# pr0g/ToyMeshPathTracer

Measured on AMD Instinct MI355X. Metric: MRays/s on sponza.obj 1920x1080 64spp at 1/2/4/8 GPUs; %HBM roofline, higher is better.
Workload: dtype f32

## Files before the change

toymeshpathtracer_amd/csrc/tmpt_aov.hip:

```cpp
#include <hip/hip_runtime.h>

#include <algorithm>
#include <string>

#include "tmpt_render.h"

namespace tmpt {

static_assert(sizeof(tmpt_aov_pixel) == 32, "AOV record: two 16-byte stores");

constexpr int kAovTicket = 8;

struct AovSample {
    f3 n;
    float t, lc;
    uint32_t flags;
    int32_t tri;
};

template <int BLOCK, int SL>
__device__ __forceinline__ AovSample aov_sample(const SceneView& sv, const RenderArgs& a, uint32_t x, uint32_t y,
                                                uint32_t smp, uint32_t& rays, uint32_t& srays,
                                                TravStack<BLOCK, SL>& st, TravCount& cnt)
{
// ... 107 lines not shown
{
    auto fn = k_aov<G, kBlk, kSL>;
    const int resident = occupancy_grid((const void*)fn, kBlk, 0, s.device);
    int grid = (int)std::max<int64_t>(1, std::min<int64_t>(resident, (a.slots * G + kBlk - 1) / kBlk));
    const size_t ovf_bytes = (size_t)grid * kBlk * (kStackTotal - kSL) * sizeof(uint32_t);
    if (ensure_ws(s, ovf_bytes)) return -1;
    fn<<<grid, kBlk, 0, s.stream>>>(view(s), a, reinterpret_cast<float4*>(d_out), (uint32_t*)s.ws, s.counters);
    TMPT_HIP(hipGetLastError());
    return 0;
}

int render_aov(Scene& s, const tmpt_camera* cam, const tmpt_render_desc* d, tmpt_aov_pixel* d_out,
               uint64_t* ray_count)
{
    RenderArgs a = make_args(cam, d);
    s.row_render = false;
    if (int rc = ensure_sample_tables(s, a.spp, "tmpt_render_aov")) return rc;
    a.jt = s.jt;
    if (int rc = wait_caller_stream(s, d, "tmpt_render_aov")) return rc;
    if (ensure_counters(s)) return -1;
    a.root_check = camera_root_check(s, a.cam);
    TMPT_HIP(hipMemsetAsync(s.counters, 0, kRenderCounters * sizeof(unsigned long long), s.stream));
    hipEvent_t e0 = s.render_ev[0], e1 = s.render_ev[1];
    TMPT_HIP(hipEventRecord(e0, s.stream));
    reset_render_stats(s);
    int rc = 0;
    if (a.slots > 0) {
        switch (s.opt.aov_group ? s.opt.aov_group : aov_auto_group(a.spp)) {
        case 1: rc = launch_aov<1>(s, a, d_out); break;
        case 2: rc = launch_aov<2>(s, a, d_out); break;
        case 4: rc = launch_aov<4>(s, a, d_out); break;
// ... 33 lines not shown
```

toymeshpathtracer_amd/csrc/tmpt_api.cpp:

```cpp
#include <dlfcn.h>
#include <hip/hip_runtime.h>
#include <rccl/rccl.h>
#include <string.h>

#include <algorithm>
#include <new>
#include <chrono>
#include <string>
#include <thread>
#include <vector>

#include "tmpt.h"
#include "tmpt_internal.h"
#include "tmpt_traverse.h"
#include "tmpt_render.h"

namespace tmpt {

static thread_local std::string g_last_error;
void set_error(const std::string& msg) { g_last_error = msg; }
const char* last_error() { return g_last_error.c_str(); }

int load_obj(const char* path, std::vector<float>& tris, f3& bmin, f3& bmax);
void camera_init(tmpt_camera* cam, f3 lookFrom, f3 lookAt, f3 vup, float vfov, float aspect,
// ... 79 lines not shown
    {"sbuf_pair", false, 0, 1, &Options::sbuf_pair, nullptr, nullptr},
    {"pilot", false, -1, 512, &Options::pilot, nullptr, nullptr},
    {"help", false, -1, 1, &Options::help, nullptr, nullptr},
    {"pair", false, -1, 63, &Options::pair, nullptr, nullptr},
    {"balance", false, 0, 1, &Options::balance, nullptr, nullptr},
    {"dprio", false, 0, 1, &Options::dprio, nullptr, nullptr},
    {"wave_cap", false, 0, 64, &Options::wave_cap, nullptr, nullptr},
    {"pixel_chains", false, -1, 1024, &Options::pixel_chains, nullptr, nullptr},
    {"tie_defer", false, -1, 1, &Options::tie_defer, nullptr, nullptr},
    {"redo_cap", false, 0, 1 << 30, &Options::redo_cap, nullptr, nullptr},
    {"redo_inline", false, 0, 1, &Options::redo_inline, nullptr, nullptr},
    {"redo_lanes", false, 1, 64, &Options::redo_lanes, nullptr, nullptr},
    {"path_waves", false, 0, 5, &Options::path_waves, nullptr, nullptr},
    {"top_walk", false, -1, 8, &Options::top_walk, nullptr, nullptr},
    {"shadow_order", false, -1, 2, &Options::shadow_order, nullptr, nullptr},
    {"rowspec", false, 0, 1, &Options::rowspec, nullptr, nullptr},
    {"rowspec_wmax", false, 0, 16384, &Options::rowspec_wmax, nullptr, nullptr},
    {"rowspec_windows", false, 0, 32, &Options::rowspec_windows, nullptr, nullptr},
    {"rowspec_spread", false, -1, 100, nullptr, &Options::rowspec_spread, nullptr},
    {"rowspec_groups", false, 1, kRowSpecMaxGroups, &Options::rowspec_groups, nullptr, nullptr},
    {"rowspec_noshadow", false, 0, 1, &Options::rowspec_noshadow, nullptr, nullptr},
    {"rowspec_chase", false, 0, 1, &Options::rowspec_chase, nullptr, nullptr},
    {"rowspec_stream", false, 0, 1, &Options::rowspec_stream, nullptr, nullptr},
    {"rowstream_dynamic", false, 0, 1, &Options::rowstream_dynamic, nullptr, nullptr},
    {"row_flag_leaves", false, 0, 1, &Options::row_flag_leaves, nullptr, nullptr},
    {"row_occ", false, 0, 5, &Options::row_occ, nullptr, nullptr},
    {"wf_bins", false, 1, 8, &Options::wf_bins, nullptr, nullptr},
    {"rowstream_test_abort", false, 0, 1, &Options::rowstream_test_abort, nullptr, nullptr},
    {"tie_rule", false, 0, 1, &Options::tie_rule, nullptr, nullptr},
    {"aov_group", false, 0, 16, &Options::aov_group, nullptr, nullptr},
// ... 429 lines not shown
    TMPT_GUARD_END
}

int tmpt_scene_set_option(tmpt_scene* h, const char* key, double value)
{
    TMPT_GUARD_BEGIN
    if (!h) return bad("tmpt_scene_set_option: null scene");
    return options_set(h->s.opt, key, value, false);
    TMPT_GUARD_END
}

int tmpt_scene_get_option(const tmpt_scene* h, const char* key, double* value)
{
    TMPT_GUARD_BEGIN
    if (!h || !value) return bad("tmpt_scene_get_option: null argument");
    return options_get(h->s.opt, key, value);
    TMPT_GUARD_END
}

namespace {
int scene_hit(const tmpt_scene* hc, const float* rays, int64_t n, float tmin, float tmax, bool ranged,
              int32_t any_hit, float* hits, int32_t* ids)
{
    if (!hc || n < 0 || (n > 0 && (!rays || !hits || !ids))) return bad("tmpt_scene_hit: bad arguments");
    if (n == 0) return 0;
    const size_t rs = ranged ? 32 : 24;
    Scene& s = const_cast<tmpt_scene*>(hc)->s;
    TMPT_HIP(hipSetDevice(s.device));
    float *d_rays = nullptr, *d_hits = nullptr;
    int32_t* d_ids = nullptr;
// ... 483 lines not shown
```

toymeshpathtracer_amd/csrc/tmpt_bvh.hip:

```cpp
#include <hip/hip_runtime.h>

#include <stdlib.h>

#include <algorithm>
#include <string>
#include <chrono>
#include <functional>
#include <cmath>
#include <mutex>
#include <thread>
#include <vector>

#include "tmpt_internal.h"

namespace tmpt {

namespace {

constexpr int kBlock = 256;

__device__ __forceinline__ uint32_t f2ord(float f)
{
    uint32_t u = __float_as_uint(f);
    return (u & 0x80000000u) ? ~u : (u | 0x80000000u);
// ... 461 lines not shown
            stn[sp] = c.y; stj[sp] = cj - k; ++sp;
            cn = c.x;
            cj = k;
        }
    }
    return no;
}

__global__ void __launch_bounds__(kBlock) k_bvh4_level(const int2* __restrict__ child,
                                                       const int2* __restrict__ range, Soa6 leaf,
                                                       const uint32_t* __restrict__ vals, Soa6 ib,
                                                       const int2* __restrict__ frontier, int nf,
                                                       int2* __restrict__ next,
                                                       uint32_t* __restrict__ counters,
                                                       Bvh4Node* __restrict__ out, int leaf_max,
                                                       int n_tris, const uint32_t* __restrict__ dec)
{
    int i = blockIdx.x * kBlock + threadIdx.x;
    if (i >= nf) return;
    const int src = frontier[i].x, dst = frontier[i].y;
    int cand[4];
    int nc;
    auto count_of = [&](int c) { return c < 0 ? 1 : range[c].y - range[c].x + 1; };
    auto is_leaf = [&](int c) { return dec ? (c < 0 || (dec[c] & 1u)) : count_of(c) <= leaf_max; };
    if (src < 0 || (dec ? (dec[src] & 1u) != 0 : count_of(src) <= leaf_max)) {
        cand[0] = src;
        nc = 1;
    } else if (dec) {
        const int2 c = child[src];
        const int k4 = (int)((dec[src] >> 1) & 3u);
        nc = sah_expand(child, dec, c.x, k4, cand);
// ... 27 lines not shown
        for (int a = 0; a < 3; ++a) {
            lo[a] = fminf(lo[a], bx[k][a]);
            hi[a] = fmaxf(hi[a], bx[k][3 + a]);
        }
    }
    uint32_t ebits = 0, mask = 0;
    uint32_t qlo[3] = {0, 0, 0}, qhi[3] = {0, 0, 0};
    double scale[3];
    for (int a = 0; a < 3; ++a) {
        double ext = (double)hi[a] - (double)lo[a];
        int e = (int)ceil(log2(fmax(ext, 1e-30) / 255.0));
        e = max(-126, min(127, e));
        scale[a] = ldexp(1.0, e);
        ebits |= ((uint32_t)e & 0xFFu) << (8 * a);
    }
    const int null_leaf = (int)(0x80000000u | (uint32_t)n_tris);
    int4 links = make_int4(null_leaf, null_leaf, null_leaf, null_leaf);
    int* lk = &links.x;
    for (int k = nc; k < 4; ++k)
        for (int a = 0; a < 3; ++a) qlo[a] |= 255u << (8 * k);
    for (int k = 0; k < nc; ++k) {
        for (int a = 0; a < 3; ++a) {
            double l = floor(((double)bx[k][a] - (double)lo[a]) / scale[a]);
            double h = ceil(((double)bx[k][3 + a] - (double)lo[a]) / scale[a]);
            uint32_t ql = (uint32_t)fmin(fmax(l, 0.0), 255.0);
            uint32_t qh = (uint32_t)fmin(fmax(h, 0.0), 255.0);
            qlo[a] |= ql << (8 * k);
            qhi[a] |= qh << (8 * k);
        }
        mask |= 1u << k;
        int c = cand[k];
        if (c < 0) {
            lk[k] = (int)(0x80000000u | (uint32_t)(~c));
        } else if (is_leaf(c)) {
            lk[k] = (int)(0x80000000u | ((uint32_t)(count_of(c) - 1) << kLeafCountShift) |
                          (uint32_t)range[c].x);
        } else {
            uint32_t slot = atomicAdd(&counters[0], 1u);
            uint32_t qi = atomicAdd(&counters[1], 1u);
            next[qi] = make_int2(c, (int)slot);
            lk[k] = (int)slot;
        }
    }
    out[dst].a = f4(lo[0], lo[1], lo[2], __uint_as_float(ebits | (mask << 24)));
    out[dst].b = make_uint4(qlo[0], qhi[0], qlo[1], qhi[1]);
    out[dst].c = make_uint4(qlo[2], qhi[2], 0u, 0u);
    out[dst].d = links;
}

__global__ void __launch_bounds__(kBlock) k_tri_pre(const float* __restrict__ tris9, int32_t n,
                                                    const uint32_t* __restrict__ vals,
// ... 113 lines not shown
}

size_t radix_sort_hist_words(int32_t n) { return 256 * (size_t)std::max(1, blocks_for(n, kSortTile)); }

namespace {

template <class Alloc>
int collapse_bvh4(Scene& s, const float* d_tris9, const int2* tchild, const int2* trange, Soa6 leaf,
                  const uint32_t* tvals, Soa6 tib, int troot, int2* fr0, int2* fr1, uint32_t* c4, Alloc& alloc)
{
    const int32_t n = s.n, m = s.n_nodes;
    hipStream_t st = s.stream;
    k_tri_pre<<<blocks_for(n, kBlock), kBlock, 0, st>>>(d_tris9, n, tvals, s.tri_pre);
    const int leaf_max = s.opt.leaf_max;
    s.leaf_max = leaf_max;
    const bool sah = s.opt.collapse == 1 && n >= 2;
    uint32_t* dec = nullptr;
    if (sah) {
        const SahCost cost{1.0f, s.opt.sah_c_leaf, s.opt.sah_c_tri};
        int32_t* ord = (int32_t*)alloc((size_t)m * 4);
        float4* Fc = (float4*)alloc((size_t)m * sizeof(float4));
        dec = (uint32_t*)alloc((size_t)m * 4);
        if (!ord || !Fc || !dec) return -1;
        std::vector<int> off = {0, 1};
        uint32_t zero = 0, cnt = 0;
        if (hipMemcpyAsync(ord, &troot, 4, hipMemcpyHostToDevice, st) != hipSuccess) return -1;
        while (off.back() > off[off.size() - 2]) {
            const int b0 = off[off.size() - 2], b1 = off.back();
            if (hipMemcpyAsync(c4, &zero, 4, hipMemcpyHostToDevice, st) != hipSuccess) return -1;
            k_bfs_level<<<blocks_for(b1 - b0, kBlock), kBlock, 0, st>>>(tchild, ord + b0, b1 - b0, ord + b1, c4);
// ... 1 lines not shown
                hipStreamSynchronize(st) != hipSuccess) return -1;
            off.push_back(b1 + (int)cnt);
        }
        for (int L = (int)off.size() - 3; L >= 0; --L)
            k_sah_level<<<blocks_for(off[L + 1] - off[L], kBlock), kBlock, 0, st>>>(
                tchild, trange, leaf, tvals, tib, ord + off[L], off[L + 1] - off[L], Fc, dec, leaf_max, cost);
    }
    int2 root = make_int2(troot, 0);
    uint32_t hc[2] = {1u, 0u};
    if (hipMemcpyAsync(fr0, &root, sizeof(root), hipMemcpyHostToDevice, st) != hipSuccess ||
        hipMemcpyAsync(c4, hc, sizeof(hc), hipMemcpyHostToDevice, st) != hipSuccess) return -1;
    int nf = 1, levels = 0;
    int2 *fa = fr0, *fb = fr1;
    while (nf > 0) {
        k_bvh4_level<<<blocks_for(nf, kBlock), kBlock, 0, st>>>(tchild, trange, leaf, tvals, tib, fa, nf,
                                                                fb, c4, s.nodes4, leaf_max, n, dec);
        ++levels;
        if (hipMemcpyAsync(hc, c4, sizeof(hc), hipMemcpyDeviceToHost, st) != hipSuccess ||
            hipStreamSynchronize(st) != hipSuccess) return -1;
        nf = (int)hc[1];
        hc[1] = 0;
        if (hipMemcpyAsync(c4 + 1, &hc[1], 4, hipMemcpyHostToDevice, st) != hipSuccess) return -1;
        std::swap(fa, fb);
        s.n_nodes4 = (int32_t)hc[0];
        s.depth4 = levels;
        if (3 * levels + 1 > kStackTotal) return 1;
    }
    return 0;
}

}
// ... 191 lines not shown
```

toymeshpathtracer_amd/csrc/tmpt_internal.h:

```cpp
#pragma once

#include <hip/hip_runtime.h>
#include <stdint.h>

#include <string>
#include <vector>

#include "tmpt_math.h"

namespace tmpt {

struct alignas(16) Bvh4Node {
    float4 a;
    uint4 b;
    uint4 c;
    int4 d;
};
static_assert(sizeof(Bvh4Node) == 64, "BVH4Q node is one half cache line");

constexpr int kLeafCountShift = 27;
constexpr uint32_t kLeafFirstMask = (1u << kLeafCountShift) - 1u;
constexpr int kLeafMaxTris = 16;
constexpr int kTopNodes = 120;
constexpr int kTopNodes5 = 80;

struct alignas(16) TriPre {
    float4 a;
    float4 b;
    float4 c;
};
struct alignas(16) TriOrig {
    float4 a;
    float4 b;
    float4 c;
};

struct alignas(16) OctNode {
// ... 40 lines not shown
    const uint4* __restrict__ na = nullptr;
    const uint4* __restrict__ nb = nullptr;
    const uint2* __restrict__ nc = nullptr;
    const int4* __restrict__ nd = nullptr;
    const float4* __restrict__ ta = nullptr;
    const float4* __restrict__ tb = nullptr;
    const float2* __restrict__ tc = nullptr;
};

constexpr float kBoxPadRel = 1e-5f;
constexpr float kTfarSlack = 1.00001f;

constexpr int kStackTotal = 128;

constexpr int kShadowOrderDefault = 2;

constexpr int kRowSpecMaxGroups = 8;
constexpr int kRenderCounters = 48;
constexpr int kTopCounter = 32;
constexpr int kTieCounter = 24;
constexpr int kCrackCounter = 30;
constexpr int kRedoRaysCounter = 31;
constexpr int kRedoCounter = 26;

struct Options {
    int builder = 0;
    int layout = 0;
    int leaf_max = 2;
    int collapse = 0;
    int ploc_radius = 32;
    float sah_c_leaf = 0.7f, sah_c_tri = 0.5f;
    int sample_block = 0;
    int rowstream_dynamic = 1;
// ... 15 lines not shown
    float rowspec_spread = -1.0f;
    int rowspec_groups = 2;
    int rowspec_noshadow = 1;
    int rowspec_chase = 1;
    int rowspec_stream = 1;
    int rowstream_test_abort = 0;
    int wf_bins = 1;
    int tie_rule = 0;
    int tie_defer = -1;
    int redo_cap = 0;
    int redo_lanes = 4;
    int path_waves = 0;
    int redo_inline = 1;
    int top_walk = -1;
    int shadow_order = -1;
    int aov_group = 0;
    int denoise_lds = -1;
};
int options_parse(Options& o, const char* text, bool allow_build);
int options_set(Options& o, const char* key, double value, bool allow_build);
int options_get(const Options& o, const char* key, double* value);

struct Scene {
    int device = 0;
    int32_t n = 0;
    int32_t n_nodes = 0;
    int32_t max_depth = 0;
    Bvh4Node* nodes4 = nullptr;
    int32_t n_nodes4 = 0, depth4 = 0, leaf_max = 0, ploc_iters = 0;
    TriPre* tri_pre = nullptr;
    TriOrig* tri_orig = nullptr;
    void* soa_buf = nullptr;
    SoaScene soa;
    std::vector<float> tris_host;
    OctNode* oct = nullptr;
    int32_t* oct_refs = nullptr;
    OctView* oct_view = nullptr;
    int32_t n_oct = 0, oct_leaves = 0, oct_depth = 0;
    int32_t oct_flat = 0;
    OctGrid oct_grid{};
    int64_t n_oct_refs = 0;
    double oct_build_ms = 0.0;
    float oct_lo[3] = {0, 0, 0}, oct_hi[3] = {0, 0, 0};
    unsigned long long* ties = nullptr;
// ... 14 lines not shown
    size_t prog_slots = 0;
    int32_t prog_key[7] = {0, 0, 0, 0, 0, 0, -1};
    uint64_t prog_cam = 0;
    uint32_t* jt = nullptr;
    int32_t jt_spp = 0;
    float4* sbuf = nullptr;
    size_t sbuf_bytes = 0;
    uint2* redo = nullptr;
    uint32_t redo_cap = 0;
    float4* redo_state = nullptr;
    int64_t redo_samples = 0;
    int64_t redo_late = 0;
    int32_t redo_launches = 0;
    int32_t tie_path = 0;
    bool row_render = false;
    double redo_ms = 0.0;
    uint64_t redo_rays = 0;
    uint32_t* jt2 = nullptr;
    int32_t jt2_n = 0;
    void* rs_buf = nullptr;
    size_t rs_bytes = 0;
    hipStream_t rs_stream[kRowSpecMaxGroups] = {};
    hipEvent_t rs_event[kRowSpecMaxGroups + 1] = {};
    uint32_t* rs_host = nullptr;
    void* rs_list = nullptr;
    size_t rs_list_bytes = 0;
    void* rss_buf = nullptr;
    size_t rss_bytes = 0;
    uint32_t* rss_tab = nullptr;
    uint32_t* rss_host = nullptr;
// ... 37 lines not shown
```

toymeshpathtracer_amd/csrc/tmpt_render.hip:

```cpp
#include <hip/hip_runtime.h>

#include <stdio.h>
#include <stdlib.h>
#include <string.h>

#include <algorithm>
#include <chrono>
#include <cmath>
#include <vector>

#include "tmpt_render.h"

namespace tmpt {

__device__ __forceinline__ uint64_t wballot(bool p) { return __builtin_amdgcn_ballot_w64(p); }
__device__ __forceinline__ bool wany(bool p) { return __builtin_amdgcn_ballot_w64(p) != 0; }

__device__ __forceinline__ uint64_t stamp()
{
    uint64_t t;
    __builtin_amdgcn_sched_barrier(0);
    asm volatile("s_memtime %0\n\ts_waitcnt lgkmcnt(0)" : "=s"(t)::"memory");
    __builtin_amdgcn_sched_barrier(0);
    return t;
// ... 1446 lines not shown
                    }
                    if (COUNT) {
                        tv_n += (uint64_t)__popcll(tm);
                        tv_lead += (uint64_t)__popcll(wballot(top && lead));
                    }
                    if (top) {
                        bool done;
                        if (!COUNT) {
                            done = trav_step4q2_mixed<false, BLOCK, SL, true, 1, SOA, false, FLAG, true>(sv, r, qany, ts, st,
                                                                                                        cnt);
                        } else {
                            TravCount c1;
                            done = trav_step4q2_mixed<COUNT, BLOCK, SL, true, 1, SOA, false, FLAG, true>(sv, r, qany, ts, st,
                                                                                                        c1);
                            (qany ? cnt_s : cnt).nodes += c1.nodes;
                        }
                        if (done) in_query = false;
                        if ((kFull && pc.cost_out) || dp0 > 0.0f) ++psteps;
                    }
                }
                if (PROF) {
                    pt_t = stamp();
                    pt_top += pt_t - tw_t;
                }
            }
        }
        if (dp0 > 0.0f) {
            float rem = 0.0f;
            if (has_pix)
                rem = smp > (uint32_t)a.smp_begin
// ... 53 lines not shown
                const bool stepping = in_query && ((ts.node < 0) == leaf_round);
                bool done = false;
                if (leaf_round) {
                    if (stepping) done = trav_step4q2_mixed<false, BLOCK, SL, true, 2, SOA, false, FLAG>(sv, r, qany, ts, st, cnt);
                } else {
                    if (stepping) done = trav_step4q2_mixed<false, BLOCK, SL, true, 1, SOA, false, FLAG>(sv, r, qany, ts, st, cnt);
                }
                if (done) in_query = false;
                if (stepping && ((kFull && pc.cost_out) || dp0 > 0.0f)) ++psteps;
            } else if (in_query && (ts.node < 0) == leaf_round) {
                TravCount c1;
                if (trav_step4q2_mixed<COUNT, BLOCK, SL, true, 0, SOA, false, FLAG>(sv, r, qany, ts, st, c1)) in_query = false;
                TravCount& dst = qany ? cnt_s : cnt;
                dst.nodes += c1.nodes;
                dst.tris += c1.tris;
                if ((kFull && pc.cost_out) || dp0 > 0.0f) ++psteps;
            }
            if (PROF) {
                const uint64_t t = stamp();
                (leaf_round ? pt_leaf : pt_node) += t - pt_t;
                if (!leaf_round) {
                    ++pn_all;
                    if ((at_node & ~top_m) != 0) {
                        ++pn_g;
                        pt_node_g += t - pt_t;
                    }
                }
                pt_t = t;
            }
        }
// ... 46 lines not shown
        }
    }
#ifdef TMPT_EXP_WAVETIME
    if (lane_id() == 0 && wt_id < kWaveTimeMax) g_wavetime[3 * wt_id + 2] = __builtin_amdgcn_s_memrealtime();
#endif
    if (SAMP == 4 && lane_id() == 0) {
        atomicAdd(&pc.rss.ctl[5], n_claim);
        atomicAdd(&pc.rss.ctl[6], n_miss);
        atomicAdd(&pc.rss.ctl[7], n_cas);
    }
    uint32_t re = wave_sum(rays_e), rs = wave_sum(rays_s);
    uint32_t nv = COUNT ? wave_sum(cnt.nodes) : 0u;
    uint32_t nt = COUNT ? wave_sum(cnt.tris) : 0u;
    uint32_t nvs = COUNT ? wave_sum(cnt_s.nodes) : 0u;
    uint32_t nts = COUNT ? wave_sum(cnt_s.tris) : 0u;
    if (lane_id() == 0) {
        atomicAdd(&counters[0], (unsigned long long)(re + rs));
        atomicAdd(&counters[3], (unsigned long long)re);
        if (COUNT) {
            atomicAdd(&counters[1], (unsigned long long)nv);
            atomicAdd(&counters[2], (unsigned long long)nt);
            atomicAdd(&counters[4], (unsigned long long)nvs);
            atomicAdd(&counters[5], (unsigned long long)nts);
        }
        if (COUNT || PROF >= 3) {
            atomicAdd(&counters[6], (unsigned long long)rs_nr);
            atomicAdd(&counters[7], (unsigned long long)rs_nl);
            atomicAdd(&counters[8], (unsigned long long)rs_lr);
            atomicAdd(&counters[9], (unsigned long long)rs_ll);
            atomicAdd(&counters[10], (unsigned long long)rs_sr);
            atomicAdd(&counters[11], (unsigned long long)rs_sl);
            atomicAdd(&counters[12], (unsigned long long)rs_st);
        }
        if (PROF) {
// ... 402 lines not shown
    if (s.ws_bytes >= bytes) return 0;
    if (s.ws) (void)hipFree(s.ws);
    s.ws = nullptr;
    s.ws_bytes = 0;
    TMPT_HIP(hipMalloc(&s.ws, bytes));
    s.ws_bytes = bytes;
    return 0;
}

static float shadow_order_weight(const Options& o, bool row)
{
    const int order = o.shadow_order >= 0 ? o.shadow_order : row ? 0 : kShadowOrderDefault;
    return order == 0 ? 0.0f : order == 1 ? -1.0f : -1024.0f;
}

SceneView view(const Scene& s)
{
    SceneView v{s.nodes4, s.tri_pre, s.tri_orig, s.n, s.n_nodes4};
    v.soa = s.soa;
    v.any_w = shadow_order_weight(s.opt, s.row_render);
#ifdef TMPT_CHECK
    v.chk = s.chk;
    if (const char* e = getenv("TMPT_CHECK_SELFTEST"))
        if (atoi(e) == 1) v.n_nodes4 = std::min(v.n_nodes4, 1);
#endif
    if (s.oct && s.opt.tie_rule == 0) {
        v.oct = s.oct_view;
        const OctGrid& g = s.oct_grid;
        v.crack = make_float4(g.reach, g.drift[0], g.drift[1], g.drift[2]);
    }
    return v;
}

namespace {

// ... 1190 lines not shown
             "32 triangle id), %u times, last value %d",
             what, h[0], h[1], (int)h[2]);
    fprintf(stderr, "tmpt: %s\n", msg);
    set_error(msg);
    return kCheckError;
#else
    (void)s;
    (void)what;
    return 0;
#endif
}

int intersect_batch(Scene& s, const float* d_rays, int64_t n, float tmin, float tmax, bool any, bool ranged,
                    float* d_hits, int32_t* d_ids)
{
    s.row_render = false;
    if (ensure_counters(s)) return -1;
    TMPT_HIP(hipMemsetAsync(s.ties, 0, 2 * sizeof(unsigned long long), s.stream));
    TMPT_HIP(hipMemsetAsync(s.counters + kCrackCounter, 0, sizeof(unsigned long long), s.stream));
    const bool soa = s.soa.na != nullptr;
    const bool neg1 = !ranged && tmin < 0.0f;
    auto fn = soa ? (ranged ? (any ? k_intersect<true, true, kBlk, kSL, true> : k_intersect<false, true, kBlk, kSL, true>)
                    : neg1  ? (any ? k_intersect<true, false, kBlk, kSL, true, true>
                                   : k_intersect<false, false, kBlk, kSL, true, true>)
                            : (any ? k_intersect<true, false, kBlk, kSL, true> : k_intersect<false, false, kBlk, kSL, true>))
                  : (ranged ? (any ? k_intersect<true, true, kBlk, kSL> : k_intersect<false, true, kBlk, kSL>)
                    : neg1  ? (any ? k_intersect<true, false, kBlk, kSL, false, true>
                                   : k_intersect<false, false, kBlk, kSL, false, true>)
                            : (any ? k_intersect<true, false, kBlk, kSL> : k_intersect<false, false, kBlk, kSL>));
    int grid = occupancy_grid((const void*)fn, kBlk, 0, s.device);
    grid = (int)std::max<int64_t>(1, std::min<int64_t>(grid, (n + kBlk - 1) / kBlk));
// ... 73 lines not shown
__global__ void __launch_bounds__(256) k_radiance_scale(float4* __restrict__ px, int64_t n, float spp_recip)
{
    const int64_t i = (int64_t)blockIdx.x * 256 + threadIdx.x;
    if (i >= n) return;
    const float4 c = px[i];
    const f3 col = mk(c.x, c.y, c.z) * spp_recip;
    px[i] = make_float4(col.x, col.y, col.z, 1.0f);
}

int render(Scene& s, const tmpt_camera* cam, const tmpt_render_desc* d, uint32_t* d_out,
           uint64_t* ray_count, float4* d_sums)
{
    RenderArgs a = make_args(cam, d);
    bool count = (d->flags & TMPT_FLAG_COUNT_VISITS) != 0;
    s.row_render = d->seed_mode == TMPT_SEED_ROW;
    const bool progressive = a.smp_begin > 0 || a.smp_end < a.spp;
    if (progressive) {
        const int32_t key[6] = {d->width, d->height, d->spp, a.band_rows, a.shard, a.nshards};
        uint64_t cam_key = 1469598103934665603ull;
        const unsigned char* cb = reinterpret_cast<const unsigned char*>(cam);
        for (size_t i = 0; i < sizeof(tmpt_camera); ++i) cam_key = (cam_key ^ cb[i]) * 1099511628211ull;
        cam_key = (cam_key ^ (uint32_t)d->seed_mode) * 1099511628211ull;
        if (a.smp_begin > 0 &&
            (memcmp(key, s.prog_key, sizeof(key)) != 0 || s.prog_key[6] != a.smp_begin || s.prog_cam != cam_key)) {
            set_error("tmpt_render: spp_begin does not continue the previous pass of this shard "
                      "(same camera, size, spp and shard)");
            return -22;
        }
        s.prog_cam = cam_key;
        if (s.prog_slots < (size_t)a.slots) {
// ... 151 lines not shown
                fprintf(stderr, "  cycles per round: node %.0f (%.1f lanes), leaf %.0f (%.1f lanes), shading %.0f "
                                "(%.1f lanes shading, %.1f traversing); rounds node %llu leaf %llu shading %llu\n",
                        (double)c[14] / c[6], (double)c[7] / c[6], (double)c[15] / c[8], (double)c[9] / c[8],
                        (double)c[13] / c[10], (double)c[11] / c[10], (double)c[12] / c[10], c[6], c[8], c[10]);
            if (c[16] + c[17] + c[18] + c[19])
                fprintf(stderr, "  shading split: ballots+pixel fetch %.1f%%, shade/finish %.1f%%, camera %.1f%%, "
                                "query set-up %.1f%% (of all wave time)\n",
                        100.0 * c[16] / tot, 100.0 * c[17] / tot, 100.0 * c[18] / tot, 100.0 * c[19] / tot);
        }
        if (count && getenv("TMPT_ROUND_LOG"))
            fprintf(stderr,
                    "k_path rounds: node %llu (%.1f lanes), leaf %llu (%.1f lanes), shade %llu "
                    "(%.1f wanting, %.1f traversing)\n",
                    c[6], c[6] ? (double)c[7] / c[6] : 0.0, c[8], c[8] ? (double)c[9] / c[8] : 0.0,
                    c[10], c[10] ? (double)c[11] / c[10] : 0.0, c[10] ? (double)c[12] / c[10] : 0.0);
        {
            const unsigned long long* t = c + kTopCounter;
            const unsigned long long nv = c[1] + c[4];
            if (count && getenv("TMPT_ROUND_LOG") && nv)
                fprintf(stderr,
                        "k_path top levels: %.4f of node lane-steps on an LDS node, %.4f of those before the query's "
                        "first other step (%.2f per query); voted node rounds with LDS lanes %.4f, of them mixed "
                        "with global lanes %.4f; top-walk rounds %llu (%.1f lanes)\n",
                        (double)t[0] / nv, t[0] ? (double)t[1] / t[0] : 0.0, (double)t[1] / (double)c[0],
                        c[6] ? (double)(t[2] + t[3]) / c[6] : 0.0, t[2] + t[3] ? (double)t[2] / (t[2] + t[3]) : 0.0,
                        t[4], t[4] ? (double)t[5] / t[4] : 0.0);
            if (t[9])
                fprintf(stderr,
                        "  node rounds with a global-side lane: %llu of %llu, %.0f cycles each; without: %.0f cycles "
                        "each; top-walk rounds %llu (%.1f lanes), %.0f cycles each, %.2f%% of wave time\n",
// ... 25 lines not shown
```

toymeshpathtracer_amd/csrc/tmpt_traverse.h:

```cpp
#pragma once

#include "tmpt_internal.h"

namespace tmpt {

__device__ __forceinline__ float safe_inv(float d)
{
    float a = fabsf(d) < 1e-20f ? copysignf(1e-20f, d) : d;
    return __builtin_amdgcn_rcpf(a);
}

struct TravRay {
    f3 o, d;
    float ix, iy, iz;
    float ox, oy, oz;
    uint32_t offx, offy, offz;
};

__device__ __forceinline__ TravRay make_trav_ray(f3 o, f3 d)
{
    TravRay r;
    r.o = o;
    r.d = d;
    r.ix = safe_inv(d.x);
// ... 19 lines not shown
                 "+v"(b.w), "+v"(c.x), "+v"(c.y));
}

typedef float v2f __attribute__((ext_vector_type(2)));
typedef __attribute__((address_space(3))) uint32_t lds_u32;
typedef uint32_t u32x4 __attribute__((ext_vector_type(4)));
typedef __attribute__((address_space(3))) u32x4 lds_u4;

template <int BLOCK, int SL>
struct TravStack {
    lds_u32* lds;
    uint32_t* glob;
    const lds_u4* top = nullptr;
    uint32_t ntop = 0;
    __device__ __forceinline__ TravStack(uint32_t* l, uint32_t* g) : lds((lds_u32*)l), glob(g) {}
    __device__ __forceinline__ void push(int& sp, int v)
    {
        if (SL >= kStackTotal || sp < SL) lds[sp * BLOCK] = (uint32_t)v;
        else glob[sp - SL] = (uint32_t)v;
        ++sp;
    }
    __device__ __forceinline__ void push3(int& sp, bool v0, int c0, bool v1, int c1, bool v2, int c2)
    {
        if (sp + 3 <= SL) {
            const int s0 = v0 ? c0 : (v1 ? c1 : c2);
            const int s1 = (v0 && v1) ? c1 : c2;
            lds[sp * BLOCK] = (uint32_t)s0;
            lds[(sp + 1) * BLOCK] = (uint32_t)s1;
            lds[(sp + 2) * BLOCK] = (uint32_t)c2;
            sp += (int)v0 + (int)v1 + (int)v2;
        } else {
            if (v0) push(sp, c0);
            if (v1) push(sp, c1);
            if (v2) push(sp, c2);
        }
    }
    __device__ __forceinline__ int pop(int& sp)
    {
        --sp;
        if (SL >= kStackTotal) return (int)lds[sp * BLOCK];
        uint32_t v = lds[min(sp, SL - 1) * BLOCK];
        if (sp >= SL) v = glob[sp - SL];
        return (int)v;
    }
};

struct SceneView {
    const Bvh4Node* __restrict__ nodes4;
    const TriPre* __restrict__ tri_pre;
    const TriOrig* __restrict__ tri_orig;
    int32_t n;
    int32_t n_nodes4 = 0;
    const OctView* __restrict__ oct = nullptr;
    float4 crack = make_float4(0.0f, 0.0f, 0.0f, 0.0f);
    SoaScene soa;
    float any_w = 0.0f;
#ifdef TMPT_CHECK
    uint32_t* chk = nullptr;
#endif
};

#ifdef TMPT_CHECK
__device__ __noinline__ void chk_fail(uint32_t* chk, uint32_t code, int what)
{
    if (chk == nullptr) return;
    __hip_atomic_fetch_or(&chk[0], code, __ATOMIC_RELAXED, __HIP_MEMORY_SCOPE_AGENT);
    __hip_atomic_fetch_add(&chk[1], 1u, __ATOMIC_RELAXED, __HIP_MEMORY_SCOPE_AGENT);
    __hip_atomic_store(&chk[2], (uint32_t)what, __ATOMIC_RELAXED, __HIP_MEMORY_SCOPE_AGENT);
}
#define TMPT_CHK(chk, ok, code, what) (__builtin_expect(!(ok), 0) && (chk_fail((chk), (code), (int)(what)), true))
#define TMPT_CHK_PARAMS , uint32_t *chk, int64_t n_refs, int32_t n_tri
#define TMPT_CHK_ARGS(sv) , (sv).chk, (sv).oct->n_refs, (sv).n
#else
#define TMPT_CHK(chk, ok, code, what) false
#define TMPT_CHK_PARAMS
#define TMPT_CHK_ARGS(sv)
#endif

struct TravCount {
    uint32_t nodes = 0, tris = 0;
};

struct TravState {
    int node;
    int sp;
    int best;
    float bt, bu, bv;
};

__device__ __forceinline__ void trav_init(TravState& ts, float tmax)
{
    ts.node = 0;
    ts.sp = 0;
    ts.best = -1;
    ts.bt = tmax;
    ts.bu = ts.bv = 0.0f;
}

template <bool COUNT, int BLOCK, int SL, bool TOPC = false, int KIND = 0, bool SOA = false, bool NEG = false,
          bool FLAG = false, bool TOPONLY = false>
__device__ __forceinline__ bool trav_step4q2_mixed(const SceneView& sv, const TravRay& r, bool any,
                                                   TravState& ts, TravStack<BLOCK, SL>& st,
                                                   TravCount& cnt, float tlo = 0.0f, float tmin = kMinT,
                                                   float tmax = kMaxT)
{
    if (KIND == 1 || (KIND == 0 && ts.node >= 0)) {
        if (TMPT_CHK(sv.chk, (uint32_t)ts.node < (uint32_t)sv.n_nodes4, kChkNode, ts.node)) return true;
        uint4 A, B, C;
        int4 L;
        if (!TOPONLY && SOA && (!TOPC || (uint32_t)ts.node >= st.ntop)) {
            const uint32_t k = (uint32_t)ts.node;
// ... 51 lines not shown
            float tf = fminf(fminf(tfx[k], tfy[k]), fminf(tfz[k], ts.bt));
            const float tf_slack = NEG ? tf + fabsf(tf) * (kTfarSlack - 1.0f) : tf * kTfarSlack;
            key[k] = tn <= tf_slack ? __builtin_fmaf(w, tf, tn) : INFINITY;
        }
        {
            const bool s01 = key[1] < key[0], s23 = key[3] < key[2];
            const float ka = s01 ? key[1] : key[0], kao = s01 ? key[0] : key[1];
            const int ca = s01 ? ch[1] : ch[0], cao = s01 ? ch[0] : ch[1];
            const float kb = s23 ? key[3] : key[2], kbo = s23 ? key[2] : key[3];
            const int cb = s23 ? ch[3] : ch[2], cbo = s23 ? ch[2] : ch[3];
            const bool sab = kb < ka;
            const float kn = sab ? kb : ka, kno = sab ? ka : kb;
            const int cn = sab ? cb : ca, cno = sab ? ca : cb;
            if (kn != INFINITY) {
                if (TMPT_CHK(sv.chk, ts.sp + 3 <= kStackTotal, kChkStack, ts.sp)) return true;
                st.push3(ts.sp, kbo != INFINITY, cbo, kao != INFINITY, cao, kno != INFINITY, cno);
                ts.node = cn;
                return false;
            }
        }
    }
    if (KIND == 2 || (KIND == 0 && ts.node < 0)) {
        const uint32_t code = (uint32_t)ts.node;
        const uint32_t first = code & kLeafFirstMask;
        const uint32_t n = ((code >> kLeafCountShift) & 15u) + 1u;
        if (TMPT_CHK(sv.chk, first + n <= (uint32_t)sv.n + 1u, kChkLeaf, code)) return true;
        const char* base = reinterpret_cast<const char*>(sv.tri_pre);
        auto tri = [&](const float4& a, const float4& b, const float4& c) -> bool {
            if (COUNT) ++cnt.tris;
            float t, u, v;
            if (mt_test(r.o, r.d, mk(a.x, a.y, a.z), mk(a.w, b.x, b.y), mk(b.z, b.w, c.x), tmin, tmax,
                        t, u, v)) {
                const int id = __float_as_int(c.y);
                const bool tie = t == ts.bt;
                if (t < ts.bt || (!FLAG && tie && id < ts.best)) {
                    ts.bt = t;
                    ts.bu = u;
                    ts.bv = v;
                    ts.best = id | (int)tie;
                    if (any) return true;
// ... 43 lines not shown
            ts.best = (acc1 ? id1 : ts.best) | (int)tie1;
            if (any && (acc0 || acc1)) return true;
        } else {
            if (tri(a0, b0, c0)) return true;
            if (n > 1u && tri(a1, b1, c1)) return true;
        }
        for (uint32_t k = 2; k < n; ++k) {
            if (SOA) {
                const float2 q = sv.soa.tc[first + k];
                if (tri(sv.soa.ta[first + k], sv.soa.tb[first + k], make_float4(q.x, q.y, 0.0f, 0.0f))) return true;
            } else {
                const float4* p = reinterpret_cast<const float4*>(base + (first + k) * (uint32_t)sizeof(TriPre));
                if (tri(p[0], p[1], p[2])) return true;
            }
        }
        if (KIND == 2 && ts.sp <= SL) {
            const uint32_t top = st.lds[(uint32_t)max(ts.sp - 1, 0) * BLOCK];
            const bool done = ts.sp == 0;
            ts.node = (int)top;
            ts.sp -= done ? 0 : 1;
            return done;
        }
    }
    if (ts.sp == 0) return true;
    ts.node = st.pop(ts.sp);
    return false;
}

__device__ __forceinline__ bool ref_slab(f3 o, f3 inv, float4 lo, float4 hi, float tmin, float tmax)
{
    const float oc[3] = {o.x, o.y, o.z}, ic[3] = {inv.x, inv.y, inv.z};
    const float lc[3] = {lo.x, lo.y, lo.z}, hc[3] = {hi.x, hi.y, hi.z};
#pragma unroll
    for (int c = 0; c < 3; ++c) {
        float t0 = (lc[c] - oc[c]) * ic[c], t1 = (hc[c] - oc[c]) * ic[c];
        if (ic[c] < 0.0f) {
            const float sw = t0;
            t0 = t1;
            t1 = sw;
        }
        tmin = t0 > tmin ? t0 : tmin;
// ... 204 lines not shown
```

Baseline: 10640.

## Pack truncated entry distances into BVH stack links to cull stale pops

Child links now use a scene-dependent bit layout sized to the triangle and node counts. The freed high bits of each traversal stack entry hold a truncated float entry distance. On pop, an entry whose key exceeds the current closest hit is discarded and the next one is taken instead, skipping node fetches that could not yield a closer hit. This adds pack and unpack ALU work per push and pop, and a second LDS read on the fast path. Culling drops at most one stale entry per pop.

```diff
diff --git a/toymeshpathtracer_amd/csrc/tmpt_aov.hip b/toymeshpathtracer_amd/csrc/tmpt_aov.hip
--- a/toymeshpathtracer_amd/csrc/tmpt_aov.hip
+++ b/toymeshpathtracer_amd/csrc/tmpt_aov.hip
@@ -145,7 +145,7 @@
                uint64_t* ray_count)
 {
     RenderArgs a = make_args(cam, d);
-    s.row_render = false;
+    s.row_render = s.pixel_render = false;
     if (int rc = ensure_sample_tables(s, a.spp, "tmpt_render_aov")) return rc;
     a.jt = s.jt;
     if (int rc = wait_caller_stream(s, d, "tmpt_render_aov")) return rc;
diff --git a/toymeshpathtracer_amd/csrc/tmpt_api.cpp b/toymeshpathtracer_amd/csrc/tmpt_api.cpp
--- a/toymeshpathtracer_amd/csrc/tmpt_api.cpp
+++ b/toymeshpathtracer_amd/csrc/tmpt_api.cpp
@@ -117,6 +117,8 @@
     {"path_waves", false, 0, 5, &Options::path_waves, nullptr, nullptr},
     {"top_walk", false, -1, 8, &Options::top_walk, nullptr, nullptr},
     {"shadow_order", false, -1, 2, &Options::shadow_order, nullptr, nullptr},
+    {"pop_cull", false, -1, 1, &Options::pop_cull, nullptr, nullptr},
+    {"pop_key_cap", false, -1, kPopKeyMax, &Options::pop_key_cap, nullptr, nullptr},
     {"rowspec", false, 0, 1, &Options::rowspec, nullptr, nullptr},
     {"rowspec_wmax", false, 0, 16384, &Options::rowspec_wmax, nullptr, nullptr},
     {"rowspec_windows", false, 0, 32, &Options::rowspec_windows, nullptr, nullptr},
@@ -576,6 +578,10 @@
 {
     TMPT_GUARD_BEGIN
     if (!h || !value) return bad("tmpt_scene_get_option: null argument");
+    if (key && strcmp(key, "pop_key_bits") == 0) {
+        *value = (double)pop_key_bits(h->s.link_bits, h->s.opt.pop_key_cap);
+        return 0;
+    }
     return options_get(h->s.opt, key, value);
     TMPT_GUARD_END
 }
diff --git a/toymeshpathtracer_amd/csrc/tmpt_bvh.hip b/toymeshpathtracer_amd/csrc/tmpt_bvh.hip
--- a/toymeshpathtracer_amd/csrc/tmpt_bvh.hip
+++ b/toymeshpathtracer_amd/csrc/tmpt_bvh.hip
@@ -499,7 +499,8 @@
                                                        int2* __restrict__ next,
                                                        uint32_t* __restrict__ counters,
                                                        Bvh4Node* __restrict__ out, int leaf_max,
-                                                       int n_tris, const uint32_t* __restrict__ dec)
+                                                       int n_tris, const uint32_t* __restrict__ dec,
+                                                       int count_shift)
 {
     int i = blockIdx.x * kBlock + threadIdx.x;
     if (i >= nf) return;
@@ -557,7 +558,7 @@
         scale[a] = ldexp(1.0, e);
         ebits |= ((uint32_t)e & 0xFFu) << (8 * a);
     }
-    const int null_leaf = (int)(0x80000000u | (uint32_t)n_tris);
+    const int null_leaf = (int)leaf_link(1u, (uint32_t)n_tris, count_shift);
     int4 links = make_int4(null_leaf, null_leaf, null_leaf, null_leaf);
     int* lk = &links.x;
     for (int k = nc; k < 4; ++k)
@@ -574,10 +575,9 @@
         mask |= 1u << k;
         int c = cand[k];
         if (c < 0) {
-            lk[k] = (int)(0x80000000u | (uint32_t)(~c));
+            lk[k] = (int)leaf_link(1u, (uint32_t)(~c), count_shift);
         } else if (is_leaf(c)) {
-            lk[k] = (int)(0x80000000u | ((uint32_t)(count_of(c) - 1) << kLeafCountShift) |
-                          (uint32_t)range[c].x);
+            lk[k] = (int)leaf_link((uint32_t)count_of(c), (uint32_t)range[c].x, count_shift);
         } else {
             uint32_t slot = atomicAdd(&counters[0], 1u);
             uint32_t qi = atomicAdd(&counters[1], 1u);
@@ -721,6 +721,13 @@
     k_tri_pre<<<blocks_for(n, kBlock), kBlock, 0, st>>>(d_tris9, n, tvals, s.tri_pre);
     const int leaf_max = s.opt.leaf_max;
     s.leaf_max = leaf_max;
+    const LinkLayout ll = link_layout((uint32_t)n, leaf_max, (uint32_t)m);
+    if (ll.count_shift > 27 || ll.link_bits > 31) {
+        set_error("build_lbvh: too many triangles for a 32-bit child link");
+        return -1;
+    }
+    s.count_shift = ll.count_shift;
+    s.link_bits = ll.link_bits;
     const bool sah = s.opt.collapse == 1 && n >= 2;
     uint32_t* dec = nullptr;
     if (sah) {
@@ -752,7 +759,8 @@
     int2 *fa = fr0, *fb = fr1;
     while (nf > 0) {
         k_bvh4_level<<<blocks_for(nf, kBlock), kBlock, 0, st>>>(tchild, trange, leaf, tvals, tib, fa, nf,
-                                                                fb, c4, s.nodes4, leaf_max, n, dec);
+                                                                fb, c4, s.nodes4, leaf_max, n, dec,
+                                                                ll.count_shift);
         ++levels;
         if (hipMemcpyAsync(hc, c4, sizeof(hc), hipMemcpyDeviceToHost, st) != hipSuccess ||
             hipStreamSynchronize(st) != hipSuccess) return -1;
diff --git a/toymeshpathtracer_amd/csrc/tmpt_internal.h b/toymeshpathtracer_amd/csrc/tmpt_internal.h
--- a/toymeshpathtracer_amd/csrc/tmpt_internal.h
+++ b/toymeshpathtracer_amd/csrc/tmpt_internal.h
@@ -18,9 +18,74 @@
 };
 static_assert(sizeof(Bvh4Node) == 64, "BVH4Q node is one half cache line");
 
-constexpr int kLeafCountShift = 27;
-constexpr uint32_t kLeafFirstMask = (1u << kLeafCountShift) - 1u;
 constexpr int kLeafMaxTris = 16;
+
+constexpr int kPopKeyMin = 9;
+constexpr int kPopKeyMax = 16;
+TMPT_HD constexpr int bits_for(uint32_t v)
+{
+    int b = 0;
+    for (; v; v >>= 1) ++b;
+    return b;
+}
+struct LinkLayout {
+    int count_shift;
+    int link_bits;
+};
+TMPT_HD constexpr LinkLayout link_layout(uint32_t n_tris, int leaf_max, uint32_t n_nodes4)
+{
+    const int cs = bits_for(n_tris), leaf = cs + bits_for((uint32_t)leaf_max - 1u);
+    const int node = bits_for(n_nodes4 ? n_nodes4 - 1u : 0u);
+    return LinkLayout{cs, leaf > node ? leaf : node};
+}
+TMPT_HD constexpr int pop_key_bits(int link_bits, int cap)
+{
+    int k = 31 - link_bits;
+    k = k > kPopKeyMax ? kPopKeyMax : k;
+    k = cap >= 0 && k > cap ? cap : k;
+    return k < kPopKeyMin ? 0 : k;
+}
+TMPT_HD constexpr uint32_t pop_key_mask(int k) { return k ? ((1u << k) - 1u) << (31 - k) : 0u; }
+TMPT_HD constexpr uint32_t leaf_link(uint32_t count, uint32_t first, int count_shift)
+{
+    return 0x80000000u | ((count - 1u) << count_shift) | first;
+}
+TMPT_HD constexpr uint32_t leaf_first(uint32_t link, int count_shift) { return link & ((1u << count_shift) - 1u); }
+TMPT_HD constexpr uint32_t leaf_count(uint32_t link, int count_shift)
+{
+    return ((link >> count_shift) & (uint32_t)(kLeafMaxTris - 1)) + 1u;
+}
+TMPT_HD constexpr uint32_t entry_pack(uint32_t link, uint32_t key_f32, uint32_t key_mask)
+{
+    return (key_f32 & key_mask) | link;
+}
+TMPT_HD constexpr uint32_t entry_key(uint32_t e, uint32_t key_mask) { return e & key_mask; }
+TMPT_HD constexpr uint32_t entry_link(uint32_t e, uint32_t key_mask) { return e ^ (e & key_mask); }
+
+namespace link_checks {
+constexpr LinkLayout kBench = link_layout(66453u, 2, 16700u);
+static_assert(kBench.count_shift == 17 && kBench.link_bits == 18, "bench scene: 18-bit links");
+static_assert(pop_key_bits(kBench.link_bits, -1) == 13 && pop_key_mask(13) == 0x7FFC0000u, "bench scene: bits 30..18");
+static_assert(pop_key_bits(kBench.link_bits, 9) == 9 && pop_key_mask(9) == 0x7FC00000u, "capped key");
+static_assert(pop_key_bits(kBench.link_bits, 0) == 0 && pop_key_bits(kBench.link_bits, 8) == 0 &&
+                  pop_key_mask(0) == 0u, "no key below 9 bits");
+static_assert(link_layout(66453u, 16, 9000u).link_bits == 21 && pop_key_bits(21, -1) == 10, "leaf_max 16");
+static_assert(link_layout(1u << 21, 2, 1u << 20).link_bits == 23 && pop_key_bits(23, -1) == 0, "2^21 triangles");
+static_assert(link_layout(1u << 21, 1, 1u << 21).link_bits == 22 && pop_key_bits(22, -1) == 9, "2^21, leaf_max 1");
+static_assert(pop_key_bits(link_layout(12u, 2, 5u).link_bits, -1) == 16 && pop_key_mask(16) == 0x7FFF8000u, "cap 16");
+static_assert(link_layout(3u, 1, 1000u).link_bits == 10, "node index decides");
+static_assert(link_layout((1u << 27) - 1u, 16, 1u << 26).link_bits == 31, "2^27 - 1 triangles still fit");
+constexpr uint32_t kLeaf = leaf_link(2u, 66452u, kBench.count_shift), kMask = pop_key_mask(13);
+constexpr uint32_t kTn = 0x4129999Au;
+static_assert(leaf_first(kLeaf, kBench.count_shift) == 66452u && leaf_count(kLeaf, kBench.count_shift) == 2u,
+              "leaf decode");
+static_assert(entry_link(entry_pack(kLeaf, kTn, kMask), kMask) == kLeaf, "leaf link survives its key");
+static_assert(entry_link(entry_pack(16699u, kTn, kMask), kMask) == 16699u, "node link survives its key");
+static_assert(entry_key(entry_pack(kLeaf, kTn, kMask), kMask) == 0x41280000u, "key = tn truncated (10.5 <= 10.6)");
+static_assert(entry_key(entry_pack(kLeaf, 0x7F800000u, kMask), kMask) == 0x7F800000u, "+inf stays +inf");
+static_assert(entry_pack(kLeaf, kTn, 0u) == kLeaf && entry_key(kLeaf, 0u) == 0u, "no key field: plain links");
+}
+
 constexpr int kTopNodes = 120;
 constexpr int kTopNodes5 = 80;
 
@@ -91,9 +156,11 @@
 constexpr int kStackTotal = 128;
 
 constexpr int kShadowOrderDefault = 2;
+constexpr int kPopCullSample = 1, kPopCullPixel = 1, kPopCullRow = 1;
 
 constexpr int kRowSpecMaxGroups = 8;
 constexpr int kRenderCounters = 48;
+constexpr int kWalkCounter = 42;
 constexpr int kTopCounter = 32;
 constexpr int kTieCounter = 24;
 constexpr int kCrackCounter = 30;
@@ -139,6 +206,8 @@
     int redo_inline = 1;
     int top_walk = -1;
     int shadow_order = -1;
+    int pop_cull = -1;
+    int pop_key_cap = -1;
     int aov_group = 0;
     int denoise_lds = -1;
 };
@@ -153,6 +222,7 @@
     int32_t max_depth = 0;
     Bvh4Node* nodes4 = nullptr;
     int32_t n_nodes4 = 0, depth4 = 0, leaf_max = 0, ploc_iters = 0;
+    int32_t count_shift = 0, link_bits = 31;
     TriPre* tri_pre = nullptr;
     TriOrig* tri_orig = nullptr;
     void* soa_buf = nullptr;
@@ -197,6 +267,7 @@
     int32_t redo_launches = 0;
     int32_t tie_path = 0;
     bool row_render = false;
+    bool pixel_render = false;
     double redo_ms = 0.0;
     uint64_t redo_rays = 0;
     uint32_t* jt2 = nullptr;
diff --git a/toymeshpathtracer_amd/csrc/tmpt_render.hip b/toymeshpathtracer_amd/csrc/tmpt_render.hip
--- a/toymeshpathtracer_amd/csrc/tmpt_render.hip
+++ b/toymeshpathtracer_amd/csrc/tmpt_render.hip
@@ -1484,6 +1484,8 @@
                             done = trav_step4q2_mixed<COUNT, BLOCK, SL, true, 1, SOA, false, FLAG, true>(sv, r, qany, ts, st,
                                                                                                         c1);
                             (qany ? cnt_s : cnt).nodes += c1.nodes;
+                            cnt.stale += c1.stale;
+                            cnt.stale2 += c1.stale2;
                         }
                         if (done) in_query = false;
                         if ((kFull && pc.cost_out) || dp0 > 0.0f) ++psteps;
@@ -1567,6 +1569,8 @@
                 TravCount& dst = qany ? cnt_s : cnt;
                 dst.nodes += c1.nodes;
                 dst.tris += c1.tris;
+                dst.stale += c1.stale;
+                dst.stale2 += c1.stale2;
                 if ((kFull && pc.cost_out) || dp0 > 0.0f) ++psteps;
             }
             if (PROF) {
@@ -1643,10 +1647,14 @@
     uint32_t nt = COUNT ? wave_sum(cnt.tris) : 0u;
     uint32_t nvs = COUNT ? wave_sum(cnt_s.nodes) : 0u;
     uint32_t nts = COUNT ? wave_sum(cnt_s.tris) : 0u;
+    uint32_t nst = COUNT ? wave_sum(cnt.stale) : 0u;
+    uint32_t nst2 = COUNT ? wave_sum(cnt.stale2) : 0u;
     if (lane_id() == 0) {
         atomicAdd(&counters[0], (unsigned long long)(re + rs));
         atomicAdd(&counters[3], (unsigned long long)re);
         if (COUNT) {
+            atomicAdd(&counters[kWalkCounter], (unsigned long long)nst);
+            atomicAdd(&counters[kWalkCounter + 1], (unsigned long long)nst2);
             atomicAdd(&counters[1], (unsigned long long)nv);
             atomicAdd(&counters[2], (unsigned long long)nt);
             atomicAdd(&counters[4], (unsigned long long)nvs);
@@ -2079,11 +2087,19 @@
     return order == 0 ? 0.0f : order == 1 ? -1.0f : -1024.0f;
 }
 
+static bool pop_cull_on(const Scene& s)
+{
+    if (s.opt.pop_cull >= 0) return s.opt.pop_cull != 0;
+    return (s.row_render ? kPopCullRow : s.pixel_render ? kPopCullPixel : kPopCullSample) != 0;
+}
+
 SceneView view(const Scene& s)
 {
     SceneView v{s.nodes4, s.tri_pre, s.tri_orig, s.n, s.n_nodes4};
     v.soa = s.soa;
     v.any_w = shadow_order_weight(s.opt, s.row_render);
+    v.count_shift = (uint32_t)s.count_shift;
+    v.key_mask = pop_cull_on(s) ? pop_key_mask(pop_key_bits(s.link_bits, s.opt.pop_key_cap)) : 0u;
 #ifdef TMPT_CHECK
     v.chk = s.chk;
     if (const char* e = getenv("TMPT_CHECK_SELFTEST"))
@@ -3304,7 +3320,7 @@
 int intersect_batch(Scene& s, const float* d_rays, int64_t n, float tmin, float tmax, bool any, bool ranged,
                     float* d_hits, int32_t* d_ids)
 {
-    s.row_render = false;
+    s.row_render = s.pixel_render = false;
     if (ensure_counters(s)) return -1;
     TMPT_HIP(hipMemsetAsync(s.ties, 0, 2 * sizeof(unsigned long long), s.stream));
     TMPT_HIP(hipMemsetAsync(s.counters + kCrackCounter, 0, sizeof(unsigned long long), s.stream));
@@ -3408,6 +3424,7 @@
     RenderArgs a = make_args(cam, d);
     bool count = (d->flags & TMPT_FLAG_COUNT_VISITS) != 0;
     s.row_render = d->seed_mode == TMPT_SEED_ROW;
+    s.pixel_render = d->seed_mode == TMPT_SEED_PIXEL;
     const bool progressive = a.smp_begin > 0 || a.smp_end < a.spp;
     if (progressive) {
         const int32_t key[6] = {d->width, d->height, d->spp, a.band_rows, a.shard, a.nshards};
@@ -3589,6 +3606,18 @@
                     "(%.1f wanting, %.1f traversing)\n",
                     c[6], c[6] ? (double)c[7] / c[6] : 0.0, c[8], c[8] ? (double)c[9] / c[8] : 0.0,
                     c[10], c[10] ? (double)c[11] / c[10] : 0.0, c[10] ? (double)c[12] / c[10] : 0.0);
+        if (count && getenv("TMPT_ROUND_LOG")) {
+            const unsigned long long* w = c + kWalkCounter;
+            const SceneView sv = view(s);
+            fprintf(stderr,
+                    "k_path walk: %d key bits, culling %s; per closest-hit query %.3f node visits, %.3f triangle "
+                    "tests; stale pops discarded %llu (%.4f of closest-hit node visits and discards), followed by another "
+                    "stale entry %.4f\n",
+                    pop_key_bits(s.link_bits, s.opt.pop_key_cap), sv.key_mask ? "on" : "off",
+                    c[3] ? (double)c[1] / c[3] : 0.0, c[3] ? (double)c[2] / c[3] : 0.0, w[0],
+                    c[1] + w[0] ? (double)w[0] / (double)(c[1] + w[0]) : 0.0,
+                    w[0] ? (double)w[1] / w[0] : 0.0);
+        }
         {
             const unsigned long long* t = c + kTopCounter;
             const unsigned long long nv = c[1] + c[4];
diff --git a/toymeshpathtracer_amd/csrc/tmpt_traverse.h b/toymeshpathtracer_amd/csrc/tmpt_traverse.h
--- a/toymeshpathtracer_amd/csrc/tmpt_traverse.h
+++ b/toymeshpathtracer_amd/csrc/tmpt_traverse.h
@@ -57,34 +57,38 @@
     const lds_u4* top = nullptr;
     uint32_t ntop = 0;
     __device__ __forceinline__ TravStack(uint32_t* l, uint32_t* g) : lds((lds_u32*)l), glob(g) {}
-    __device__ __forceinline__ void push(int& sp, int v)
+    __device__ __forceinline__ void push(int& sp, uint32_t e)
     {
-        if (SL >= kStackTotal || sp < SL) lds[sp * BLOCK] = (uint32_t)v;
-        else glob[sp - SL] = (uint32_t)v;
+        if (SL >= kStackTotal || sp < SL) lds[sp * BLOCK] = e;
+        else glob[sp - SL] = e;
         ++sp;
     }
-    __device__ __forceinline__ void push3(int& sp, bool v0, int c0, bool v1, int c1, bool v2, int c2)
+    __device__ __forceinline__ void push3(int& sp, uint32_t key_mask, bool v0, int c0, float k0, bool v1, int c1,
+                                          float k1, bool v2, int c2, float k2)
     {
+        const uint32_t e0 = entry_pack((uint32_t)c0, __float_as_uint(k0), key_mask);
+        const uint32_t e1 = entry_pack((uint32_t)c1, __float_as_uint(k1), key_mask);
+        const uint32_t e2 = entry_pack((uint32_t)c2, __float_as_uint(k2), key_mask);
         if (sp + 3 <= SL) {
-            const int s0 = v0 ? c0 : (v1 ? c1 : c2);
-            const int s1 = (v0 && v1) ? c1 : c2;
-            lds[sp * BLOCK] = (uint32_t)s0;
-            lds[(sp + 1) * BLOCK] = (uint32_t)s1;
-            lds[(sp + 2) * BLOCK] = (uint32_t)c2;
+            const uint32_t s0 = v0 ? e0 : (v1 ? e1 : e2);
+            const uint32_t s1 = (v0 && v1) ? e1 : e2;
+            lds[sp * BLOCK] = s0;
+            lds[(sp + 1) * BLOCK] = s1;
+            lds[(sp + 2) * BLOCK] = e2;
             sp += (int)v0 + (int)v1 + (int)v2;
         } else {
-            if (v0) push(sp, c0);
-            if (v1) push(sp, c1);
-            if (v2) push(sp, c2);
-        }
-    }
-    __device__ __forceinline__ int pop(int& sp)
+            if (v0) push(sp, e0);
+            if (v1) push(sp, e1);
+            if (v2) push(sp, e2);
+        }
+    }
+    __device__ __forceinline__ uint32_t pop(int& sp)
     {
         --sp;
-        if (SL >= kStackTotal) return (int)lds[sp * BLOCK];
+        if (SL >= kStackTotal) return lds[sp * BLOCK];
         uint32_t v = lds[min(sp, SL - 1) * BLOCK];
         if (sp >= SL) v = glob[sp - SL];
-        return (int)v;
+        return v;
     }
 };
 
@@ -98,6 +102,7 @@
     float4 crack = make_float4(0.0f, 0.0f, 0.0f, 0.0f);
     SoaScene soa;
     float any_w = 0.0f;
+    uint32_t count_shift = 27, key_mask = 0u;
 #ifdef TMPT_CHECK
     uint32_t* chk = nullptr;
 #endif
@@ -122,6 +127,7 @@
 
 struct TravCount {
     uint32_t nodes = 0, tris = 0;
+    uint32_t stale = 0, stale2 = 0;
 };
 
 struct TravState {
@@ -138,6 +144,39 @@
     ts.best = -1;
     ts.bt = tmax;
     ts.bu = ts.bv = 0.0f;
+}
+
+template <bool COUNT, int KIND, bool NEG, int BLOCK, int SL>
+__device__ __forceinline__ bool trav_pop(const SceneView& sv, bool any, TravState& ts, TravStack<BLOCK, SL>& st,
+                                         TravCount& cnt)
+{
+    const uint32_t km = NEG ? 0u : sv.key_mask;
+    const float lim = any ? INFINITY : ts.bt * kTfarSlack;
+    auto is_stale = [&](uint32_t e) { return !NEG && __uint_as_float(entry_key(e, km)) > lim; };
+    if (KIND != 0 && ts.sp <= SL) {
+        const uint32_t e1 = st.lds[(uint32_t)max(ts.sp - 1, 0) * BLOCK];
+        const uint32_t e2 = st.lds[(uint32_t)max(ts.sp - 2, 0) * BLOCK];
+        const bool stale = is_stale(e1);
+        const int take = stale ? 2 : 1;
+        const bool done = ts.sp < take;
+        if (COUNT && stale && ts.sp >= 1) {
+            ++cnt.stale;
+            if (ts.sp >= 2 && is_stale(e2)) ++cnt.stale2;
+        }
+        ts.node = (int)entry_link(stale ? e2 : e1, km);
+        ts.sp = max(ts.sp - take, 0);
+        return done;
+    }
+    if (ts.sp == 0) return true;
+    uint32_t e = st.pop(ts.sp);
+    if (is_stale(e)) {
+        if (COUNT) ++cnt.stale;
+        if (ts.sp == 0) return true;
+        e = st.pop(ts.sp);
+        if (COUNT && is_stale(e)) ++cnt.stale2;
+    }
+    ts.node = (int)entry_link(e, km);
+    return false;
 }
 
 template <bool COUNT, int BLOCK, int SL, bool TOPC = false, int KIND = 0, bool SOA = false, bool NEG = false,
@@ -219,7 +258,8 @@
             const int cn = sab ? cb : ca, cno = sab ? ca : cb;
             if (kn != INFINITY) {
                 if (TMPT_CHK(sv.chk, ts.sp + 3 <= kStackTotal, kChkStack, ts.sp)) return true;
-                st.push3(ts.sp, kbo != INFINITY, cbo, kao != INFINITY, cao, kno != INFINITY, cno);
+                st.push3(ts.sp, NEG ? 0u : sv.key_mask, kbo != INFINITY, cbo, kbo, kao != INFINITY, cao, kao,
+                         kno != INFINITY, cno, kno);
                 ts.node = cn;
                 return false;
             }
@@ -227,8 +267,8 @@
     }
     if (KIND == 2 || (KIND == 0 && ts.node < 0)) {
         const uint32_t code = (uint32_t)ts.node;
-        const uint32_t first = code & kLeafFirstMask;
-        const uint32_t n = ((code >> kLeafCountShift) & 15u) + 1u;
+        const uint32_t first = leaf_first(code, (int)sv.count_shift);
+        const uint32_t n = leaf_count(code, (int)sv.count_shift);
         if (TMPT_CHK(sv.chk, first + n <= (uint32_t)sv.n + 1u, kChkLeaf, code)) return true;
         const char* base = reinterpret_cast<const char*>(sv.tri_pre);
         auto tri = [&](const float4& a, const float4& b, const float4& c) -> bool {
@@ -302,17 +342,8 @@
                 if (tri(p[0], p[1], p[2])) return true;
             }
         }
-        if (KIND == 2 && ts.sp <= SL) {
-            const uint32_t top = st.lds[(uint32_t)max(ts.sp - 1, 0) * BLOCK];
-            const bool done = ts.sp == 0;
-            ts.node = (int)top;
-            ts.sp -= done ? 0 : 1;
-            return done;
-        }
-    }
-    if (ts.sp == 0) return true;
-    ts.node = st.pop(ts.sp);
-    return false;
+    }
+    return trav_pop<COUNT, KIND, NEG>(sv, any, ts, st, cnt);
 }
 
 __device__ __forceinline__ bool ref_slab(f3 o, f3 inv, float4 lo, float4 hi, float tmin, float tmax)
```

New measurement: 10840, median of 6. 1.02x the previous value.
